# jl6017/AutoURDF

Hardware: AMD Instinct MI355X
Metric: registered frames/sec (N=4096 pts, K=20 clusters) (higher is better)
Workload: dtype f32

## Files before the change

autourdf_amd/csrc/nn_l1.h:

```cpp
#pragma once
#include <type_traits>
#include "creg_dev.h"

namespace creg {

constexpr int NN_TCH = 4096;
constexpr int NN_BLOCK = 512;
typedef float nn_f2 __attribute__((ext_vector_type(2)));

struct NnEpilogueNone {
    __device__ __forceinline__ void finish(int, int, float, float*) const {}
    __device__ __forceinline__ void shift(int) {}
};

template <int QW, typename IdxT, typename Epi>
__device__ __forceinline__ void nn_l1_block(
    const float* A, int na, int sa, const float* B, int nb, int sb,
    float* __restrict__ dA, IdxT* __restrict__ iA, float* __restrict__ dB, IdxT* __restrict__ iB,
    int blocksA, Epi& epi, int bx) {
    extern __shared__ __attribute__((aligned(16))) char smem_raw[];
    float* sX = (float*)smem_raw;
    __shared__ float s_part[NN_BLOCK / 64];
    const int tid = threadIdx.x, lane = tid & 63;
    const int wave = __builtin_amdgcn_readfirstlane(tid >> 6);
// ... 84 lines not shown
        if (dO) { dO[q0 + lane] = mv; iO[q0 + lane] = (IdxT)mi; }
        if constexpr (!std::is_same<Epi, NnEpilogueNone>::value) {
            float tx, ty, tz;
            if (in_lds) { tx = sX[mi]; ty = sX[padded0 + mi]; tz = sX[2 * padded0 + mi]; }
            else { const float* p = T + (size_t)mi * st; tx = p[0]; ty = p[1]; tz = p[2]; }
            epi(dir, q0 + lane, mi, mv, mqx, mqy, mqz, tx, ty, tz, acc);
        }
    }
    if constexpr (!std::is_same<Epi, NnEpilogueNone>::value) {
        acc = wave_sum_fast(acc);
        if (lane == 0) s_part[wave] = acc;
        __syncthreads();
        if (tid == 0) {
            float s = 0.f;
#pragma unroll
            for (int w = 0; w < NN_BLOCK / 64; ++w) s += s_part[w];
            epi.finish(dir, blk, s, nullptr);
        }
    }
}

struct NnBlocks { const float4* ts4; const float* tbox; int nblk; const int* nblk_dev; };

template <int NB, int PPL, typename Epi, bool STOP = false, bool NBDEV = false>
__device__ __forceinline__ void nn_l1_block_pruned(const float* Q, int nq, int sq, NnBlocks tb, int dir, Epi& epi, int blk,
                                                   const int* stop_flag = nullptr, const float* T = nullptr, int st = 0) {
    constexpr int QW = 4;
    int stop = 0;
    if constexpr (STOP) stop = *stop_flag;
    __shared__ float s_partp[NN_BLOCK / 64];
    const int tid = threadIdx.x, lane = tid & 63;
    const int wave = __builtin_amdgcn_readfirstlane(tid >> 6);
    const int q0 = (blk * (NN_BLOCK / 64) + wave) * QW;
    int nblk = tb.nblk;
    if constexpr (NBDEV) nblk = *tb.nblk_dev;
    float lox[NB], loy[NB], loz[NB], hix[NB], hiy[NB], hiz[NB];
#pragma unroll
    for (int g = 0; g < NB; ++g) {
        const float* bx = tb.tbox + (NBDEV ? 64 * g + lane : min(64 * g + lane, nblk - 1));
        constexpr int BP = 64 * NB;
        lox[g] = bx[0]; loy[g] = bx[BP]; loz[g] = bx[2 * BP]; hix[g] = bx[3 * BP]; hiy[g] = bx[4 * BP]; hiz[g] = bx[5 * BP];
    }
    float qx[QW], qy[QW], qz[QW], lb[QW][NB], bd[QW], tx[QW], ty[QW], tz[QW], wb[QW];
    int bi[QW];
    unsigned long long pend[QW][NB];
#pragma unroll
    for (int u = 0; u < QW; ++u) {
        const int qi = min(q0 + u, nq - 1);
        qx[u] = Q[(size_t)qi * sq]; qy[u] = Q[(size_t)qi * sq + 1]; qz[u] = Q[(size_t)qi * sq + 2];
    }
    if constexpr (STOP || NBDEV) {
        stop = __builtin_amdgcn_readfirstlane(stop); nblk = __builtin_amdgcn_readfirstlane(nblk);
#pragma unroll
        for (int u = 0; u < QW; ++u) {
            qx[u] = __int_as_float(__builtin_amdgcn_readfirstlane(__float_as_int(qx[u])));
            qy[u] = __int_as_float(__builtin_amdgcn_readfirstlane(__float_as_int(qy[u])));
            qz[u] = __int_as_float(__builtin_amdgcn_readfirstlane(__float_as_int(qz[u])));
        }
    }
#pragma unroll
    for (int u = 0; u < QW; ++u) {
        float lm = INFINITY;
#pragma unroll
        for (int g = 0; g < NB; ++g) {
            const float ex = fmaxf(fmaxf(lox[g] - qx[u], qx[u] - hix[g]), 0.f);
            const float ey = fmaxf(fmaxf(loy[g] - qy[u], qy[u] - hiy[g]), 0.f);
            const float ez = fmaxf(fmaxf(loz[g] - qz[u], qz[u] - hiz[g]), 0.f);
            const float bound = (ex + ey) + ez;
            lb[u][g] = 64 * g + lane < nblk ? bound : INFINITY;
            lm = __builtin_fminf(lm, lb[u][g]);
        }
        const float m = wave_min_fast(lm);
        bool found = false;
#pragma unroll
        for (int g = 0; g < NB; ++g) {
            const unsigned long long f = __ballot(lb[u][g] == m && 64 * g + lane < nblk);
            pend[u][g] = (!found && f) ? (f & (~f + 1ull)) : 0ull;
            found = found || f != 0ull;
        }
        if (!found) pend[u][0] = 1ull;
        bd[u] = INFINITY; bi[u] = 0x7fffffff; tx[u] = ty[u] = tz[u] = 0.f; wb[u] = INFINITY;
    }
    if (stop) return;
    bool more = true;
    while (more) {
        int b[QW];
        bool act[QW];
#pragma unroll
        for (int u = 0; u < QW; ++u) {
            b[u] = 0; act[u] = false;
#pragma unroll
            for (int g = NB - 1; g >= 0; --g)
                if (pend[u][g]) { b[u] = 64 * g + __builtin_ctzll(pend[u][g]); act[u] = true; }
        }
        float4 v1[QW];
        if constexpr (PPL == 1) {
#pragma unroll
            for (int u = 0; u < QW; ++u) v1[u] = tb.ts4[(size_t)b[u] * 64 + lane];
        }
        more = false;
#pragma unroll
        for (int u = 0; u < QW; ++u) {
            if (act[u]) {
                float4 v[PPL];
                if constexpr (PPL == 1) v[0] = v1[u];
                else {
#pragma unroll
                    for (int k = 0; k < PPL; ++k) v[k] = tb.ts4[((size_t)b[u] * PPL + k) * 64 + lane];
                }
#pragma unroll
                for (int g = 0; g < NB; ++g)
                    if ((b[u] >> 6) == g && lane == (b[u] & 63)) lb[u][g] = INFINITY;
                if constexpr (PPL > 1) {
                    unsigned long long key = ((unsigned long long)__float_as_uint(bd[u]) << 32) | (unsigned)bi[u];
#pragma unroll
                    for (int k = 0; k < PPL; ++k) {
                        const float d = l1_dist(qx[u], qy[u], qz[u], v[k].x, v[k].y, v[k].z);
                        const unsigned long long kk = ((unsigned long long)__float_as_uint(d) << 32) | (unsigned)__float_as_int(v[k].w);
                        key = kk < key ? kk : key;
                    }
                    bd[u] = __uint_as_float((unsigned)(key >> 32)); bi[u] = (int)(unsigned)key;
                } else {
#pragma unroll
                    for (int k = 0; k < PPL; ++k) {
                        const float d = l1_dist(qx[u], qy[u], qz[u], v[k].x, v[k].y, v[k].z);
                        const int oi = __float_as_int(v[k].w);
                        const unsigned long long key = ((unsigned long long)__float_as_uint(bd[u]) << 32) | (unsigned)bi[u];
                        const unsigned long long kk = ((unsigned long long)__float_as_uint(d) << 32) | (unsigned)oi;
                        const bool take = kk < key;
                        bd[u] = take ? d : bd[u]; bi[u] = take ? oi : bi[u];
                        tx[u] = take ? v[k].x : tx[u]; ty[u] = take ? v[k].y : ty[u]; tz[u] = take ? v[k].z : tz[u];
                    }
                }
                wb[u] = wave_min_fast(bd[u]);
#pragma unroll
                for (int g = 0; g < NB; ++g) {
                    pend[u][g] = __ballot(lb[u][g] <= wb[u] && lb[u][g] < INFINITY);
                    more |= pend[u][g] != 0ull;
                }
            }
        }
    }
    float acc = 0.f, mv = 0.f, mqx = 0.f, mqy = 0.f, mqz = 0.f, mtx = 0.f, mty = 0.f, mtz = 0.f;
    int mi = 0;
#pragma unroll
    for (int u = 0; u < QW; ++u) {
        const int i = wave_min_fast(bd[u] == wb[u] ? bi[u] : 0x7fffffff);
        const unsigned long long win = __ballot(bd[u] == wb[u] && bi[u] == i);
        const int src = win ? __builtin_ctzll(win) : 0;
        const float fx = __int_as_float(__builtin_amdgcn_readlane(__float_as_int(tx[u]), src));
        const float fy = __int_as_float(__builtin_amdgcn_readlane(__float_as_int(ty[u]), src));
        const float fz = __int_as_float(__builtin_amdgcn_readlane(__float_as_int(tz[u]), src));
        if (lane == u) { mv = wb[u]; mi = i; mqx = qx[u]; mqy = qy[u]; mqz = qz[u]; mtx = fx; mty = fy; mtz = fz; }
    }
    if constexpr (PPL > 1) {
        if (lane < QW && q0 + lane < nq && mi != 0x7fffffff) { const float* p = T + (size_t)mi * st; mtx = p[0]; mty = p[1]; mtz = p[2]; }
    }
    if (lane < QW && q0 + lane < nq) epi(dir, q0 + lane, mi, mv, mqx, mqy, mqz, mtx, mty, mtz, acc);
    acc = wave_sum_fast(acc);
    if (lane == 0) s_partp[wave] = acc;
    __syncthreads();
    if (tid == 0) {
        float s = 0.f;
#pragma unroll
        for (int w = 0; w < NN_BLOCK / 64; ++w) s += s_partp[w];
        epi.finish(dir, blk, s, nullptr);
    }
}

__device__ __forceinline__ float row_min16(float v) {
    asm("s_nop 4\n\t"
        "v_min_f32_dpp %0, %0, %0 quad_perm:[1,0,3,2] row_mask:0xf bank_mask:0xf\n\ts_nop 1\n\t"
        "v_min_f32_dpp %0, %0, %0 quad_perm:[2,3,0,1] row_mask:0xf bank_mask:0xf\n\ts_nop 1\n\t"
        "v_min_f32_dpp %0, %0, %0 row_half_mirror row_mask:0xf bank_mask:0xf\n\ts_nop 1\n\t"
        "v_min_f32_dpp %0, %0, %0 row_mirror row_mask:0xf bank_mask:0xf\n\ts_nop 1"
        : "+v"(v));
    return v;
}
__device__ __forceinline__ float row_max16(float v) {
    asm("s_nop 4\n\t"
        "v_max_f32_dpp %0, %0, %0 quad_perm:[1,0,3,2] row_mask:0xf bank_mask:0xf\n\ts_nop 1\n\t"
// ... 238 lines not shown
```

autourdf_amd/csrc/train_engine.hip:

```cpp
#include <cfloat>
#include <chrono>
#include <cmath>
#include <cstdlib>
#include <cstring>
#include <type_traits>
#include <vector>
#include "creg_common.h"
#include "nn_l1.h"

#ifndef CREG_L2_IN_BD_DEFAULT
#define CREG_L2_IN_BD_DEFAULT false
#endif

namespace creg {

struct Dims {
    int rot, K, KP, IN, H, HA, HB, H2, OA, OB, NP, NT, epochs;
    float slope;
    int oW1, ob1, oW2, ob2, oW3A, ob3A, oW3B, ob3B, NPAR;
    int nbx, nby;
    int nyb;
    int npb;
    int ppl;
    int nbt, nbp;
    int rows;
};

constexpr int PS_MAXB = 512;

struct Hyper {
    float lr, factor;
    int patience, stop;
};

struct TrainState {
    double lr, sched_best;
    int sched_bad, count, stopped, step;
    float min_loss;
    int epochs_run, best_epoch;
    float step_size, bc2_sqrt;
    float last_loss;
    float next_bc2s;
    double next_bc1;
};

struct Ws {
    float *P, *P1, *AM, *AV;
    float *pose_in, *enc, *x1[2], *h2[2], *head_save, *m2, *gm2;
    float4 *pts4, *y4, *pred4, *ys4, *psl4, *ps4;
    float *ybox, *pbox;
    int* sb;
    int* sgn_x;
    int4* cnt4;
    float *lossp_x, *lossp_y;
    float *g_out, *g_h2;
    TrainState* state;
    double* bc1;
    float* bc2s;
    float *best_m, *best_pred, *loss_hist, *lr_hist, *result;
    int* off;
    Hyper* hyper;
    unsigned long long* ysum;
    int* sync;
};

static_assert(sizeof(Ws) % sizeof(char*) == 0, "Ws must hold pointers only");
__host__ __device__ __forceinline__ Ws ws_shift(Ws W, size_t bytes) {
    char** p = reinterpret_cast<char**>(&W);
#pragma unroll
    for (size_t i = 0; i < sizeof(Ws) / sizeof(char*); ++i) p[i] += bytes;
    return W;
}

constexpr int ROT_Q = 0, ROT_DQ = 1, ROT_6D = 2, ROT_RPY = 3;
constexpr int POSE_IN = 12;
__device__ __forceinline__ float act_f(float v, float slope) { return v > 0.f ? v : v * slope; }
__device__ __forceinline__ float act_grad(float post, float slope) { return post > 0.f ? 1.f : slope; }

__device__ __forceinline__ int seg_of(const int* __restrict__ off, int k, int n) {
    int lo = 0, hi = k;
    while (hi - lo > 1) { const int mid = (lo + hi) >> 1; if (off[mid] <= n) lo = mid; else hi = mid; }
    return lo;
}

constexpr int PREP_MAXB = 64;
struct PrepBatch { const float* m[PREP_MAXB]; const float* y[PREP_MAXB]; const float* pts[PREP_MAXB]; Hyper hy[PREP_MAXB]; };
// ... 39 lines not shown
                nin = 9;
            } else {
                in[0] = tr[0]; in[1] = tr[1]; in[2] = tr[2];
                matrix_to_euler_xyz(R, in + 3);
                nin = 6;
            }
            for (int i = 0; i < POSE_IN; ++i) W.pose_in[POSE_IN * r + i] = in[i];
            float* e = W.enc + (size_t)r * D.IN;
            for (int f = 0; f < 4; ++f) {
                const float mul = (float)(1 << f);
                for (int i = 0; i < nin; ++i) {
                    e[(2 * f) * nin + i] = sinf(mul * in[i]);
                    e[(2 * f + 1) * nin + i] = cosf(mul * in[i]);
                }
            }
        }
        if (threadIdx.x == 0) {
            TrainState s;
            *W.hyper = hy;
            s.lr = (double)hy.lr; s.sched_best = INFINITY; s.sched_bad = 0; s.count = 0; s.stopped = 0;
            s.step = 0; s.min_loss = 1000.f; s.epochs_run = 0; s.best_epoch = -1; s.step_size = 0.f;
            s.bc2_sqrt = 1.f; s.last_loss = NAN;
            s.next_bc1 = 1.0 - 0.9; s.next_bc2s = (float)sqrt(1.0 - 0.999);
            W.state[0] = s; W.state[1] = s;
            for (int i = 0; i < 64; ++i) W.sync[i] = 0;
        }
    }
}

__global__ __launch_bounds__(256) void k_l1(Dims D, Ws W0, int par, size_t bstride) {
    const Ws W = ws_shift(W0, blockIdx.z * bstride);
    const int lane = threadIdx.x & 63;
    const int o = blockIdx.x * 4 + (threadIdx.x >> 6);
    if (o >= D.H) return;
    const float w = lane < D.IN ? W.P[D.oW1 + (size_t)o * D.IN + lane] : 0.f;
    const float w2 = 64 + lane < D.IN ? W.P[D.oW1 + (size_t)o * D.IN + 64 + lane] : 0.f;
    const float b = W.P[D.ob1 + o];
    for (int r = 0; r < D.K; ++r) {
        float t = lane < D.IN ? w * W.enc[(size_t)r * D.IN + lane] : 0.f;
        if (64 + lane < D.IN) t = fmaf(w2, W.enc[(size_t)r * D.IN + 64 + lane], t);
        const float v = wave_sum_fast(t) + b;
        if (lane == 0) (par ? W.x1[1] : W.x1[0])[(size_t)r * D.H + o] = act_f(v, D.slope);
    }
}

typedef float f32x4 __attribute__((ext_vector_type(4)));
constexpr int L2_THREADS = 512;
// ... 89 lines not shown
    else { w = Pc + D.oW3B + (size_t)(o - D.OA) * D.HB; a = h2cur + (size_t)r * D.H2 + D.HA; n = D.HB; }
    float wv[NC], av[NC];
#pragma unroll
    for (int c = 0; c < NC; ++c) { const int i = min(c * 64 + lane, n - 1); wv[c] = w[i]; av[c] = a[i]; }
    const float bias = o < D.OA ? Pc[D.ob3A + o] : Pc[D.ob3B + o - D.OA];
    float wv9[NC], av9[NC], bias9 = 0.f;
    if constexpr (X) {
        const float* w9 = Pc + D.oW3B + (size_t)(8 - D.OA) * D.HB;
        const float* a9 = h2cur + (size_t)r * D.H2 + D.HA;
#pragma unroll
        for (int c = 0; c < NC; ++c) { const int i = min(c * 64 + lane, D.HB - 1); wv9[c] = w9[i]; av9[c] = a9[i]; }
        bias9 = Pc[D.ob3B + 8 - D.OA];
    }
    __builtin_amdgcn_sched_barrier(0);
    const int stopped = W.state[par].stopped;
    float pin[POSE_IN];
#pragma unroll
    for (int i = 0; i < POSE_IN; ++i) pin[i] = W.pose_in[POSE_IN * r + i];
    const int b = W.off[r], e = W.off[r + 1];
    const int BS = 64 * D.ppl;
    const int sb0 = W.sb[r], sb1 = W.sb[r + 1];
    const int s0 = D.npb ? BS * sb0 : 0, s1 = D.npb ? BS * sb1 : 0;
    const float4 p_first = D.npb ? W.psl4[min(s0 + (int)threadIdx.x, BS * D.npb - 1)] : W.pts4[min(b + (int)threadIdx.x, D.NP - 1)];
    {
        float s = 0.f;
#pragma unroll
        for (int c = 0; c < NC; ++c) s = fmaf(c * 64 + lane < n ? wv[c] : 0.f, av[c], s);
        s = wave_sum_fast(s) + bias;
        if (lane == 0 && wave < NO) outs[o] = s;
        if constexpr (X) {
            float s9 = 0.f;
#pragma unroll
            for (int c = 0; c < NC; ++c) s9 = fmaf(c * 64 + lane < D.HB ? wv9[c] : 0.f, av9[c], s9);
            s9 = wave_sum_fast(s9) + bias9;
            if (lane == 0 && wave == 0) outs[8] = s9;
        }
    }
    __syncthreads();
    if (stopped) return;
    if (threadIdx.x == 0) {
        const float* in = pin;
        float R[9], t[3], save[16];
        for (int i = 0; i < 16; ++i) save[i] = 0.f;
        if (D.rot == ROT_6D) {
            for (int i = 0; i < 3; ++i) t[i] = outs[i] + in[i];
            float d6[6];
// ... 21 lines not shown
            for (int i = 0; i < 8; ++i) save[i] = dq[i];
        }
        for (int a = 0; a < 3; ++a) { m2s[4 * a] = R[3 * a]; m2s[4 * a + 1] = R[3 * a + 1]; m2s[4 * a + 2] = R[3 * a + 2]; m2s[4 * a + 3] = t[a]; }
        for (int i = 0; i < 12; ++i) W.m2[16 * r + i] = m2s[i];
        W.m2[16 * r + 12] = 0.f; W.m2[16 * r + 13] = 0.f; W.m2[16 * r + 14] = 0.f; W.m2[16 * r + 15] = 1.f;
        for (int i = 0; i < 16; ++i) W.head_save[16 * r + i] = save[i];
    }
    __syncthreads();
    if (D.npb) {
        __shared__ float wbox[8][6];
        for (int base = s0; base < s1; base += 512) {
            const int sl = base + threadIdx.x;
            const bool in = sl < s1;
            const float4 p = !in ? make_float4(0.f, 0.f, 0.f, __int_as_float(0x7fffffff)) : (base == s0 ? p_first : W.psl4[sl]);
            const int n = __float_as_int(p.w);
            const bool real = n != 0x7fffffff;
            float o[3];
#pragma unroll
            for (int a = 0; a < 3; ++a) o[a] = fmaf(p.z, m2s[4 * a + 2], fmaf(p.y, m2s[4 * a + 1], p.x * m2s[4 * a])) + m2s[4 * a + 3];
            if (real) {
                W.pred4[n] = make_float4(o[0], o[1], o[2], 0.f);
                W.cnt4[n] = make_int4(0, 0, 0, 0);
            }
            if (in) W.ps4[sl] = real ? make_float4(o[0], o[1], o[2], p.w) : make_float4(INFINITY, INFINITY, INFINITY, p.w);
            float bx[6];
#pragma unroll
            for (int a = 0; a < 3; ++a) {
                bx[a] = wave_min_fast(real ? o[a] : INFINITY);
                bx[3 + a] = -wave_min_fast(real ? -o[a] : INFINITY);
            }
            if (D.ppl == 1) {
                if (lane == 0 && in) {
                    float* pb = W.pbox + (sl >> 6);
#pragma unroll
                    for (int a = 0; a < 6; ++a) pb[a * 64 * D.nbp] = bx[a];
                }
            } else {
                if (lane == 0) {
#pragma unroll
                    for (int a = 0; a < 6; ++a) wbox[wave][a] = bx[a];
                }
                __syncthreads();
                if (threadIdx.x < 12) {
                    const int hb = threadIdx.x / 6, a = threadIdx.x % 6;
                    if (base + 256 * hb < s1) {
                        float v = wbox[4 * hb][a];
// ... 215 lines not shown
    const int* stopped;
    __device__ __forceinline__ void shift(int z) {
        const size_t b = (size_t)z * bstride;
        sgn_x = (int*)((char*)sgn_x + b); cnt4 = (int4*)((char*)cnt4 + b);
        lossp_x = (float*)((char*)lossp_x + b); lossp_y = (float*)((char*)lossp_y + b);
        stopped = (const int*)((const char*)stopped + b);
    }
    __device__ __forceinline__ void operator()(int dir, int q, int idx, float d, float qx, float qy, float qz,
                                               float tx, float ty, float tz, float& acc) const {
        if (dir == 0) {
            sgn_x[q] = (qx > tx ? 1 : 0) | (qy > ty ? 2 : 0) | (qz > tz ? 4 : 0);
        } else {
            atomicAdd(&cnt4[idx].x, (qx > tx) ? -1 : 1);
            atomicAdd(&cnt4[idx].y, (qy > ty) ? -1 : 1);
            atomicAdd(&cnt4[idx].z, (qz > tz) ? -1 : 1);
        }
        acc += d;
    }
    __device__ __forceinline__ void finish(int dir, int blk, float s, float*) const { (dir == 0 ? lossp_x : lossp_y)[blk] = s; }
};

template <bool P1, int PPL, int NBT, int NBP>
__global__ __launch_bounds__(NN_BLOCK) void k_nn_plan(const float* A, int na, const float* B, int nb, int blocksA,
                                                      int blocksB, EngineEpi epi, NnBlocks yb, NnBlocks pb, size_t zstride) {
    asm volatile("" :: "s"(A), "s"(na), "s"(B), "s"(nb), "s"(blocksA), "s"(blocksB), "s"(epi.sgn_x), "s"(epi.cnt4), "s"(epi.lossp_x), "s"(epi.lossp_y),
                 "s"(epi.bstride), "s"(epi.stopped), "s"(yb.ts4), "s"(yb.tbox), "s"(yb.nblk), "s"(pb.ts4), "s"(pb.tbox), "s"(pb.nblk_dev), "s"(zstride));
    const int nz = gridDim.x / (blocksA + blocksB);
    int i = blockIdx.x, z, bx;
    if (i < blocksB * nz) { z = i / blocksB; bx = blocksA + (i - z * blocksB); }
    else { i -= blocksB * nz; z = i / blocksA; bx = i - z * blocksA; }
    const size_t zb = z * zstride;
    A = (const float*)((const char*)A + zb);
    B = (const float*)((const char*)B + zb);
    yb.ts4 = (const float4*)((const char*)yb.ts4 + zb);
    yb.tbox = (const float*)((const char*)yb.tbox + zb);
    epi.shift(z);
    if (bx < blocksA) nn_l1_block_pruned<NBT, PPL, EngineEpi, true, false>(A, na, 4, yb, 0, epi, bx, epi.stopped, B, 4);
    else if constexpr (P1) {
        pb.ts4 = (const float4*)((const char*)pb.ts4 + zb);
        pb.tbox = (const float*)((const char*)pb.tbox + zb);
        pb.nblk_dev = (const int*)((const char*)pb.nblk_dev + zb);
        nn_l1_block_pruned<NBP, PPL, EngineEpi, true, true>(B, nb, 4, pb, 1, epi, bx - blocksA, epi.stopped, A, 4);
    } else nn_l1_block<4, int, EngineEpi>(A, na, 4, B, nb, 4, nullptr, nullptr, nullptr, nullptr, blocksA, epi, bx);
}

template <int NBT, int NBP>
__global__ __launch_bounds__(NN_ROWS_BLOCK) void k_nn_rows(const float* A, const float* B, int blocksA, int blocksB, EngineEpi epi, NnBlocks yb, NnBlocks pb,
                                                      size_t zstride) {
    asm volatile("" :: "s"(A), "s"(B), "s"(blocksA), "s"(blocksB), "s"(epi.sgn_x), "s"(epi.cnt4), "s"(epi.lossp_x), "s"(epi.lossp_y),
                 "s"(epi.bstride), "s"(epi.stopped), "s"(yb.ts4), "s"(yb.tbox), "s"(yb.nblk), "s"(pb.ts4), "s"(pb.tbox), "s"(pb.nblk_dev), "s"(zstride));
    const int nz = gridDim.x / (blocksA + blocksB);
    int i = blockIdx.x, z, bx;
    if (i < blocksB * nz) { z = i / blocksB; bx = blocksA + (i - z * blocksB); }
    else { i -= blocksB * nz; z = i / blocksA; bx = i - z * blocksA; }
    const size_t zb = z * zstride;
    A = (const float*)((const char*)A + zb);
    B = (const float*)((const char*)B + zb);
    yb.ts4 = (const float4*)((const char*)yb.ts4 + zb);
    yb.tbox = (const float*)((const char*)yb.tbox + zb);
    pb.ts4 = (const float4*)((const char*)pb.ts4 + zb);
    pb.tbox = (const float*)((const char*)pb.tbox + zb);
    pb.nblk_dev = (const int*)((const char*)pb.nblk_dev + zb);
    epi.shift(z);
    if (bx < blocksA) nn_l1_rows<NBT, EngineEpi, false, true>(pb.ts4, 0, pb.nblk_dev, pb.nblk, yb, 0, epi, bx, epi.stopped, B, epi.lossp_x);
    else nn_l1_rows<NBP, EngineEpi, true, false>(yb.ts4, yb.nblk, nullptr, yb.nblk, pb, 1, epi, bx - blocksA, epi.stopped, A, epi.lossp_y);
// ... 19 lines not shown
        if (N.sched_bad > hy.patience) {
            const double nl = fmax(S.lr * (double)hy.factor, 0.0);
            if (S.lr - nl > 1e-8) N.lr = nl;
            N.sched_bad = 0;
        }
    }
    return N;
}

constexpr int GC_QMAX = 3;
__device__ __forceinline__ void gradc_arrive(const Ws& W) {
    asm volatile("s_waitcnt vmcnt(0)" ::: "memory");
    __syncthreads();
    if (threadIdx.x == 0) __hip_atomic_fetch_add(W.sync, 1, __ATOMIC_RELAXED, __HIP_MEMORY_SCOPE_AGENT);
}
template <bool FUSED>
__device__ __forceinline__ void gradc_role(const Dims& D, const Ws& W, int epoch, int nbx, int nby, int k) {
    __shared__ float red[4][14];
    __shared__ float s_loss;
    __shared__ float s_go[16];
    __shared__ __attribute__((aligned(16))) float s_gh[FUSED ? 256 * GC_QMAX : 4];
    const int tid = threadIdx.x, lane = tid & 63, wv = tid >> 6;
    const TrainState S = W.state[epoch & 1];
    const int handoff_err = W.sync[3];
    const int b0 = W.off[k], e0 = W.off[k + 1];
    const Hyper hy = *W.hyper;
    float a = tid < nbx ? W.lossp_x[tid] : 0.f, b = tid < nby ? W.lossp_y[tid] : 0.f;
    const float m2v = W.m2[16 * k + (tid & 15)];
    float sv[16];
#pragma unroll
    for (int i = 0; i < 16; ++i) sv[i] = W.head_save[16 * k + i];
    const float* h2cur = (epoch & 1) ? W.h2[1] : W.h2[0];
    float w3v[GC_QMAX][8], h2v[GC_QMAX];
#pragma unroll
    for (int q = 0; q < GC_QMAX; ++q) {
        const int o = min(q * 256 + tid, D.H2 - 1);
        const bool isA = o < D.HA;
        const float* Pc = (epoch & 1) ? W.P1 : W.P;
        const float* wb = isA ? Pc + D.oW3A + o : Pc + D.oW3B + (o - D.HA);
        const int stride = isA ? D.HA : D.HB, nj = isA ? D.OA : D.OB;
#pragma unroll
        for (int j = 0; j < 8; ++j) w3v[q][j] = wb[(size_t)min(j, nj - 1) * stride];
        h2v[q] = h2cur[(size_t)k * D.H2 + o];
    }
    asm volatile("" :: "v"(a), "v"(b), "v"(m2v), "v"(sv[0]), "v"(sv[1]), "v"(sv[2]), "v"(sv[3]), "v"(sv[4]), "v"(sv[5]), "v"(sv[6]), "v"(sv[7]),
                 "v"(sv[8]), "v"(sv[9]), "v"(sv[10]), "v"(sv[11]), "v"(sv[12]), "v"(sv[13]), "v"(sv[14]), "v"(sv[15]), "v"(b0), "v"(e0), "v"(hy.lr));
// ... 20 lines not shown
    for (int i = tid + 256; i < nby; i += 256) b += W.lossp_y[i];
    a = wave_sum_fast(a); b = wave_sum_fast(b);
    if (lane == 0) { red[wv][0] = a; red[wv][1] = b; }
    __syncthreads();
    if (tid == 0) {
        const float sa = ((red[0][0] + red[1][0]) + red[2][0]) + red[3][0];
        const float sb = ((red[0][1] + red[1][1]) + red[2][1]) + red[3][1];
        s_loss = sa / (float)D.NP + sb / (float)D.NT;
    }
    __syncthreads();
    const float loss = s_loss;
    TrainState N = advance_state(S, loss, hy, S.next_bc1, S.next_bc2s);
    const bool improved = loss < S.min_loss;
    if (improved) {
        for (int n = b0 + tid; n < e0; n += 256) {
            const float4 p = (n == b0 + tid) ? pr_first : W.pred4[n];
            W.best_pred[3 * (size_t)n] = p.x; W.best_pred[3 * (size_t)n + 1] = p.y; W.best_pred[3 * (size_t)n + 2] = p.z;
        }
        if (tid < 16) W.best_m[16 * k + tid] = m2v;
    }
    if (k == 0 && tid == 0) {
        N.next_bc1 = W.bc1[min(N.step + 1, D.epochs)];
        N.next_bc2s = W.bc2s[min(N.step + 1, D.epochs)];
        W.state[(epoch + 1) & 1] = N;
        W.loss_hist[S.epochs_run] = loss;
        W.lr_hist[S.epochs_run] = (float)S.lr;
        W.result[0] = N.min_loss; W.result[1] = (float)N.epochs_run; W.result[2] = (float)N.lr; W.result[3] = (float)N.best_epoch;
        if constexpr (FUSED) st4_wt((float*)W.sync, 32, make_float4(__int_as_float(N.stopped), N.step_size, N.bc2_sqrt, 0.f));
    }
    if (N.stopped) {
        if constexpr (FUSED) gradc_arrive(W);
        return;
    }
    const float gx = 1.0f / (float)D.NP, gy = 1.0f / (float)D.NT;
    float acc[12];
#pragma unroll
    for (int i = 0; i < 12; ++i) acc[i] = 0.f;
    for (int n = b0 + tid; n < e0; n += 256) {
        const bool first = n == b0 + tid;
        const float4 p = first ? p_first : W.pts4[n];
        const int4 c = first ? c_first : W.cnt4[n];
        const int sb = first ? s_first : W.sgn_x[n];
        const float g[3] = {((sb & 1) ? gx : -gx) + gy * (float)c.x, ((sb & 2) ? gx : -gx) + gy * (float)c.y,
                            ((sb & 4) ? gx : -gx) + gy * (float)c.z};
#pragma unroll
        for (int q = 0; q < 3; ++q) {
// ... 562 lines not shown
    }
    i -= nG * nz;
    const bool roleB = i < nB * nz;
    if (!roleB) i -= nB * nz;
    const int n = roleB ? nB : nD, z = i / n, blk = i - z * n;
    const Ws W = ws_shift(W0, (size_t)z * bstride);
    if (roleB) bwd2_role<KW, X, true>(D, W, epoch, blk, (float*)smem, 0ull);
    else dw_role<true>(D, W, epoch, blk, 0ull);
}

__global__ __launch_bounds__(256) void k_params_home(Dims D, Ws W0, size_t bstride, int sidx, int step0) {
    const Ws W = ws_shift(W0, blockIdx.z * bstride);
    if (((W.state[sidx].step - step0) & 1) == 0) return;
    for (int i = blockIdx.x * 256 + threadIdx.x; i < D.NPAR; i += gridDim.x * 256) W.P[i] = W.P1[i];
}

struct ResumeState { double lr, sched_best; int step, epochs_run, sched_bad, count, best_epoch, stopped; float min_loss; };
__global__ void k_set_state(Dims D, Ws W, ResumeState rs) {
    if (threadIdx.x || blockIdx.x) return;
    TrainState s = W.state[0];
    s.lr = rs.lr; s.sched_best = rs.sched_best; s.sched_bad = rs.sched_bad; s.count = rs.count; s.stopped = rs.stopped; s.step = rs.step;
    s.min_loss = rs.min_loss; s.epochs_run = rs.epochs_run; s.best_epoch = rs.best_epoch;
    s.next_bc1 = W.bc1[min(rs.step + 1, D.epochs)]; s.next_bc2s = W.bc2s[min(rs.step + 1, D.epochs)];
    W.state[0] = s; W.state[1] = s;
    W.sync[1] = (D.H / B2_CB) * rs.step;
    W.result[0] = s.min_loss; W.result[1] = (float)s.epochs_run; W.result[2] = (float)s.lr; W.result[3] = (float)s.best_epoch;
}
__global__ void k_get_state(Ws W, int sidx, double* out) {
    if (threadIdx.x || blockIdx.x) return;
    const TrainState s = W.state[sidx];
    out[0] = s.step; out[1] = s.epochs_run; out[2] = s.lr; out[3] = s.sched_best; out[4] = s.sched_bad; out[5] = s.count;
    out[6] = (double)s.min_loss; out[7] = s.best_epoch; out[8] = s.stopped; out[9] = (double)s.last_loss; out[10] = 0.0; out[11] = 0.0;
}

struct Plan {
    creg_train_shape shape;
    Dims D;
    Ws W;
    char* base;
    size_t bytes;
    hipGraphExec_t gexec;
    bool graph_ready;
    int graph_epochs;
    int B;
    int nz;
    size_t bstride;
    int smem_bd;
// ... 24 lines not shown
    D->H2 = D->HA + D->HB;
    if (sizeof(float) * b2_smem_floats(D->K, D->IN, D->H2) > 160 * 1024) return false;
    int o = 0;
    D->oW1 = o; o += D->H * D->IN; D->ob1 = o; o += D->H;
    D->oW2 = o; o += D->H2 * D->H; D->ob2 = o; o += D->H2;
    D->oW3A = o; o += D->OA * D->HA; D->ob3A = o; o += D->OA;
    D->oW3B = o; o += D->OB * D->HB; D->ob3B = o; o += D->OB;
    D->NPAR = o;
    if (D->H2 % 32 || D->H % B2_CB || D->H2 > 256 * GC_QMAX) return false;
    const NnGrid g = nn_grid(D->NP, D->NT, true, true, 4);
    D->nbx = g.blocksA; D->nby = g.blocksB;
    const bool rows_fit = D->NT <= 16384 && D->NP < 65535 && (D->NP + 63) / 64 + D->K <= PS_MAXB && g.qw == 4;
    const char* rows_env = getenv("CREG_NN_ROWS");
    const bool rows_pays = D->NT > 64 * 64;
    D->rows = s->nn_search == 0 && rows_fit && (rows_env ? rows_env[0] == '1' : rows_pays);
    D->ppl = (D->rows || D->NT <= 64 * 64) ? 1 : 4;
    const int BS = 64 * D->ppl;
    D->nyb = (s->nn_search != 1 && D->NT <= 4 * YS_CHUNK && g.qw == 4) ? (D->NT + BS - 1) / BS : 0;
    D->npb = (D->nyb && D->NP < 65535 && (D->NP + BS - 1) / BS + D->K <= PS_MAXB) ? (D->NP + BS - 1) / BS + D->K : 0;
    const int nt = (D->nyb + 63) / 64, np = (D->npb + 63) / 64;
    D->nbt = nt <= 1 ? 1 : (nt <= 2 ? 2 : 4);
    D->nbp = np <= 2 ? 2 : (np <= 3 ? 3 : (np <= 4 ? 4 : (np <= 5 ? 5 : (np <= 6 ? 6 : 8))));
    if (D->rows) { D->nbx = 4 * D->npb; D->nby = 4 * D->nyb; }
    return true;
}

static size_t carve(const Dims& D, char* base, Ws* W) {
    size_t o = 0;
    auto take = [&](size_t bytes) -> char* { char* r = base ? base + o : nullptr; o = align_up(o + bytes, 256); return r; };
    const size_t f = sizeof(float);
    Ws w;
    w.P = (float*)take(f * D.NPAR); w.P1 = (float*)take(f * D.NPAR); w.AM = (float*)take(f * D.NPAR); w.AV = (float*)take(f * D.NPAR);
    w.pose_in = (float*)take(f * POSE_IN * D.K); w.enc = (float*)take(f * D.K * D.IN);
    w.x1[0] = (float*)take(f * D.KP * D.H); w.x1[1] = (float*)take(f * D.KP * D.H);
    w.h2[0] = (float*)take(f * D.KP * D.H2); w.h2[1] = (float*)take(f * D.KP * D.H2); w.head_save = (float*)take(f * 16 * D.K);
    w.m2 = (float*)take(f * 16 * D.K); w.gm2 = (float*)take(f * 16 * D.K);
    w.pts4 = (float4*)take(sizeof(float4) * D.NP); w.y4 = (float4*)take(sizeof(float4) * D.NT);
    w.pred4 = (float4*)take(sizeof(float4) * D.NP);
    const size_t bs = 64 * (size_t)D.ppl;
    w.ys4 = (float4*)take(sizeof(float4) * bs * (D.nyb ? D.nyb : 1)); w.ybox = (float*)take(f * 6 * 64 * D.nbt);
    w.psl4 = (float4*)take(sizeof(float4) * bs * (D.npb ? D.npb : 1)); w.ps4 = (float4*)take(sizeof(float4) * bs * (D.npb ? D.npb : 1));
    w.pbox = (float*)take(f * 6 * 64 * D.nbp); w.sb = (int*)take(sizeof(int) * (D.K + 1));
    w.sgn_x = (int*)take(sizeof(int) * D.NP);
    w.cnt4 = (int4*)take(sizeof(int4) * D.NP);
    w.lossp_x = (float*)take(f * D.nbx); w.lossp_y = (float*)take(f * D.nby);
    w.g_out = (float*)take(f * 16 * D.KP); w.g_h2 = (float*)take(f * D.KP * D.H2);
    w.state = (TrainState*)take(sizeof(TrainState) * 2);
    w.bc1 = (double*)take(sizeof(double) * (D.epochs + 1)); w.bc2s = (float*)take(f * (D.epochs + 1));
    w.best_m = (float*)take(f * 16 * D.K); w.best_pred = (float*)take(f * 3 * D.NP);
    w.loss_hist = (float*)take(f * D.epochs); w.lr_hist = (float*)take(f * D.epochs); w.result = (float*)take(f * 4);
    w.off = (int*)take(sizeof(int) * (D.K + 1)); w.hyper = (Hyper*)take(sizeof(Hyper));
    w.sync = (int*)take(sizeof(int) * 64);
    w.ysum = (unsigned long long*)take(sizeof(unsigned long long) * 4);
    if (W) *W = w;
    return o;
}

template <typename F>
static void by_nc(int H, F f) {
    switch (H / 64) {
        case 1: f(std::integral_constant<int, 1>{}); break;
        case 2: f(std::integral_constant<int, 2>{}); break;
        case 4: f(std::integral_constant<int, 4>{}); break;
        default: f(std::integral_constant<int, 8>{}); break;
    }
}
static void launch_l2(Plan* P, int par, hipStream_t s) {
    const Dims& D = P->D; const Ws& W = P->W;
    by_nc(D.H, [&](auto nc) {
        hipLaunchKernelGGL((k_l2<decltype(nc)::value>), dim3(D.H2 / 16, 1, P->nz), dim3(L2_THREADS), 0, s, D, W, par, P->bstride); });
}
static void launch_head(Plan* P, int par, hipStream_t s) {
    const Dims& D = P->D; const Ws& W = P->W;
    by_nc(D.H, [&](auto nc) {
        if (D.OA + D.OB > 8) hipLaunchKernelGGL((k_head<decltype(nc)::value, true>), dim3(D.K, 1, P->nz), dim3(512), 0, s, D, W, par, P->bstride);
        else hipLaunchKernelGGL((k_head<decltype(nc)::value>), dim3(D.K, 1, P->nz), dim3(512), 0, s, D, W, par, P->bstride);
// ... 41 lines not shown
        auto go = [&](auto kern) {
            hipLaunchKernelGGL(kern, grid, dim3(NN_ROWS_BLOCK), 0, s, (const float*)W.pred4, (const float*)W.y4, blocksA, blocksB, epi, yb, pb, bstride);
        };
        auto pick_p = [&](auto nbt) {
            constexpr int NBT = decltype(nbt)::value;
            switch (D.nbp) {
                case 2: go(k_nn_rows<NBT, 2>); break;
                case 3: go(k_nn_rows<NBT, 3>); break;
                case 4: go(k_nn_rows<NBT, 4>); break;
                case 5: go(k_nn_rows<NBT, 5>); break;
                case 6: go(k_nn_rows<NBT, 6>); break;
                default: go(k_nn_rows<NBT, 8>); break;
            }
        };
        switch (D.nbt) {
            case 1: pick_p(std::integral_constant<int, 1>{}); break;
            case 2: pick_p(std::integral_constant<int, 2>{}); break;
            default: pick_p(std::integral_constant<int, 4>{}); break;
        }
    } else if (D.nyb) {
        const NnGrid g = nn_grid(D.NP, D.NT, true, true, 4);
        const NnBlocks yb{W.ys4, W.ybox, D.nyb, nullptr}, pb{W.ps4, W.pbox, 0, W.sb + D.K};
        const dim3 grid((g.blocksA + g.blocksB) * nz);
        auto go = [&](auto kern, int smem) {
            hipLaunchKernelGGL(kern, grid, dim3(NN_BLOCK), smem, s, (const float*)W.pred4, D.NP, (const float*)W.y4, D.NT,
                               g.blocksA, g.blocksB, epi, yb, pb, bstride);
        };
        auto pick_p = [&](auto ppl, auto nbt) {
            constexpr int PPL = decltype(ppl)::value, NBT = decltype(nbt)::value;
            if (!D.npb) { go(k_nn_plan<false, PPL, NBT, 2>, g.smem); return; }
            switch (D.nbp) {
                case 2: go(k_nn_plan<true, PPL, NBT, 2>, 0); break;
                case 3: go(k_nn_plan<true, PPL, NBT, 3>, 0); break;
                case 4: go(k_nn_plan<true, PPL, NBT, 4>, 0); break;
                case 5: go(k_nn_plan<true, PPL, NBT, 5>, 0); break;
                case 6: go(k_nn_plan<true, PPL, NBT, 6>, 0); break;
                default: go(k_nn_plan<true, PPL, NBT, 8>, 0); break;
            }
        };
        auto pick_t = [&](auto ppl) {
            switch (D.nbt) {
                case 1: pick_p(ppl, std::integral_constant<int, 1>{}); break;
                case 2: pick_p(ppl, std::integral_constant<int, 2>{}); break;
                default: pick_p(ppl, std::integral_constant<int, 4>{}); break;
            }
        };
        if (D.ppl == 1) pick_t(std::integral_constant<int, 1>{}); else pick_t(std::integral_constant<int, 4>{});
    } else {
        launch_nn_l1<int>((const float*)W.pred4, D.NP, 4, (const float*)W.y4, D.NT, 4, nullptr, nullptr, nullptr, nullptr,
// ... 550 lines not shown
    for (auto& e : ev) (void)hipEventDestroy(e);
    return CREG_OK;
}

#ifdef CREG_BD_STAMPS
extern "C" int creg_debug_bd_stamps(double* out) {
    BdStamps* z = new BdStamps;
    if (hipMemcpyFromSymbol(z, HIP_SYMBOL(g_bd_st), sizeof(*z)) != hipSuccess) { delete z; return CREG_EHIP; }
    for (int i = 0; i < 24; ++i) out[i] = 0.0;
    int n = 0;
    for (int sl = 0; sl < 256; ++sl) {
        if (z->first[sl] == ~0ull || !z->endB[sl] || !z->endD[sl]) continue;
        ++n;
        const double f = (double)z->first[sl];
        out[0] += ((double)(z->endB[sl] > z->endD[sl] ? z->endB[sl] : z->endD[sl]) - f) / 100.0;
        out[1] += ((double)z->startB[sl] - f) / 100.0; out[2] += ((double)z->endB[sl] - f) / 100.0;
        out[3] += ((double)z->startD[sl] - f) / 100.0; out[4] += ((double)z->endD[sl] - f) / 100.0;
    }
    for (int i = 0; i < 5; ++i) out[i] /= n ? n : 1;
    out[5] = n ? (double)z->blocks[0] / n : 0; out[6] = n ? (double)z->blocks[1] / n : 0; out[7] = n;
    for (int r = 0; r < 2; ++r)
        for (int k = 0; k < 8; ++k) out[8 + 8 * r + k] = z->blocks[r] ? (double)z->phase[r][k] / (double)z->blocks[r] / 100.0 : 0.0;
    delete z;
    return CREG_OK;
}
#endif

#ifdef CREG_NN_STATS
extern "C" int creg_debug_nn_stats(unsigned long long* out8, int reset) {
    CREG_HIP(hipMemcpyFromSymbol(out8, HIP_SYMBOL(creg::g_nn_stats), sizeof(unsigned long long) * 8));
    if (reset) { unsigned long long z[8] = {0}; CREG_HIP(hipMemcpyToSymbol(HIP_SYMBOL(creg::g_nn_stats), z, sizeof(z))); }
    return CREG_OK;
}
#endif

#ifdef CREG_NN_WAVE_STAMPS
extern "C" long long creg_debug_nn_waves(unsigned long long* out, long long cap, int reset) {
    static unsigned n[creg::NN_WAVE_SHARDS * 32];
    if (hipMemcpyFromSymbol(n, HIP_SYMBOL(creg::g_nn_wave_n), sizeof(n)) != hipSuccess) return -1;
    long long total = 0;
    if (out && cap > 0) {
        std::vector<creg::NnWaveRec> h((size_t)creg::NN_WAVE_CAP);
        if (hipMemcpyFromSymbol(h.data(), HIP_SYMBOL(creg::g_nn_wave), sizeof(creg::NnWaveRec) * (size_t)creg::NN_WAVE_CAP) != hipSuccess) return -1;
        for (unsigned sh = 0; sh < creg::NN_WAVE_SHARDS; ++sh) {
            const unsigned m = n[32 * sh] < creg::NN_WAVE_PER ? n[32 * sh] : creg::NN_WAVE_PER;
            for (unsigned i = 0; i < m && total < cap; ++i, ++total) {
// ... 287 lines not shown
```

Baseline: 165.5.

## Certify nearest-neighbor matches across epochs to skip pruned search

```diff
diff --git a/autourdf_amd/csrc/nn_l1.h b/autourdf_amd/csrc/nn_l1.h
--- a/autourdf_amd/csrc/nn_l1.h
+++ b/autourdf_amd/csrc/nn_l1.h
@@ -130,12 +130,32 @@
 
 struct NnBlocks { const float4* ts4; const float* tbox; int nblk; const int* nblk_dev; };
 
-template <int NB, int PPL, typename Epi, bool STOP = false, bool NBDEV = false>
+struct NnCert {
+    float4* ref;
+    int* j;
+    const int* ok;
+    const double* s;
+    const unsigned* delta;
+    int nt;
+};
+__device__ __forceinline__ double nn_cert_s(int ok, double s_prev, unsigned delta_bits) {
+    return ok ? (s_prev + (double)__uint_as_float(delta_bits)) * (1.0 + 0x1p-50) : 0.0;
+}
+#ifdef CREG_NN_CERT_STATS
+__device__ unsigned long long g_nn_cert_stats[8];
+#endif
+
+template <int NB, int PPL, typename Epi, bool STOP = false, bool NBDEV = false, bool CERT = false>
 __device__ __forceinline__ void nn_l1_block_pruned(const float* Q, int nq, int sq, NnBlocks tb, int dir, Epi& epi, int blk,
-                                                   const int* stop_flag = nullptr, const float* T = nullptr, int st = 0) {
+                                                   const int* stop_flag = nullptr, const float* T = nullptr, int st = 0, NnCert cert = {}) {
     constexpr int QW = 4;
+    static_assert(!CERT || PPL == 1, "certified matches: one point per lane");
     int stop = 0;
     if constexpr (STOP) stop = *stop_flag;
+    int cok = 0;
+    double cs_prev = 0.0;
+    unsigned cdelta = 0u;
+    if constexpr (CERT) { cok = *cert.ok; cs_prev = *cert.s; cdelta = *cert.delta; }
     __shared__ float s_partp[NN_BLOCK / 64];
     const int tid = threadIdx.x, lane = tid & 63;
     const int wave = __builtin_amdgcn_readfirstlane(tid >> 6);
@@ -166,8 +186,43 @@
             qz[u] = __int_as_float(__builtin_amdgcn_readfirstlane(__float_as_int(qz[u])));
         }
     }
+    unsigned long long cmask = 0ull;
+    const double cS = CERT ? nn_cert_s(cok, cs_prev, cdelta) : 0.0;
+    float b2[QW];
+    float cd = 0.f, ctx = 0.f, cty = 0.f, ctz = 0.f;
+    int cj = 0;
+    if constexpr (CERT) {
+        if (cok) {
+            const int cq = min(q0 + min(lane, QW - 1), nq - 1);
+            const float4 r = cert.ref[cq];
+            const int j0 = cert.j[cq];
+            const float4 qv = ((const float4*)Q)[cq];
+            const bool jin = j0 >= 0 && j0 < cert.nt;
+            const float4 tv = ((const float4*)T)[jin ? j0 : 0];
+            const float d = l1_dist(qv.x, qv.y, qv.z, tv.x, tv.y, tv.z);
+            const double A = dir == 0 ? (fabs((double)qv.x - (double)r.x) + fabs((double)qv.y - (double)r.y)) + fabs((double)qv.z - (double)r.z)
+                                      : cS - __hiloint2double(__float_as_int(r.y), __float_as_int(r.x));
+            const double R = (double)r.w * (1.0 - 0x1p-20) - A * (1.0 + 0x1p-40);
+            cmask = __ballot(lane < QW && q0 + lane < nq && jin && r.w <= 0x1p126f && (double)d < R);
+            cd = d; cj = j0; ctx = tv.x; cty = tv.y; ctz = tv.z;
+        }
+#ifdef CREG_NN_CERT_STATS
+        if (lane == 0 && !stop) {
+            const int nv = min(QW, nq - q0), nc = __builtin_popcountll(cmask);
+            atomicAdd(&g_nn_cert_stats[4 * dir], 1ull); atomicAdd(&g_nn_cert_stats[4 * dir + 1], (unsigned long long)nv);
+            atomicAdd(&g_nn_cert_stats[4 * dir + 2], (unsigned long long)nc);
+            if (nc == nv) atomicAdd(&g_nn_cert_stats[4 * dir + 3], 1ull);
+        }
+#endif
+    }
 #pragma unroll
     for (int u = 0; u < QW; ++u) {
+        b2[u] = INFINITY;
+        if (CERT && ((cmask >> u) & 1ull)) {
+#pragma unroll
+            for (int g = 0; g < NB; ++g) { lb[u][g] = INFINITY; pend[u][g] = 0ull; }
+            continue;
+        }
         float lm = INFINITY;
 #pragma unroll
         for (int g = 0; g < NB; ++g) {
@@ -190,7 +245,7 @@
         bd[u] = INFINITY; bi[u] = 0x7fffffff; tx[u] = ty[u] = tz[u] = 0.f; wb[u] = INFINITY;
     }
     if (stop) return;
-    bool more = true;
+    bool more = !CERT || cmask != (1ull << QW) - 1;
     while (more) {
         int b[QW];
         bool act[QW];
@@ -236,6 +291,7 @@
                         const unsigned long long key = ((unsigned long long)__float_as_uint(bd[u]) << 32) | (unsigned)bi[u];
                         const unsigned long long kk = ((unsigned long long)__float_as_uint(d) << 32) | (unsigned)oi;
                         const bool take = kk < key;
+                        if constexpr (CERT) b2[u] = take ? bd[u] : __builtin_fminf(b2[u], d);
                         bd[u] = take ? d : bd[u]; bi[u] = take ? oi : bi[u];
                         tx[u] = take ? v[k].x : tx[u]; ty[u] = take ? v[k].y : ty[u]; tz[u] = take ? v[k].z : tz[u];
                     }
@@ -249,10 +305,14 @@
             }
         }
     }
-    float acc = 0.f, mv = 0.f, mqx = 0.f, mqy = 0.f, mqz = 0.f, mtx = 0.f, mty = 0.f, mtz = 0.f;
+    float acc = 0.f, mv = 0.f, mqx = 0.f, mqy = 0.f, mqz = 0.f, mtx = 0.f, mty = 0.f, mtz = 0.f, cL = 0.f;
     int mi = 0;
 #pragma unroll
     for (int u = 0; u < QW; ++u) {
+        if (CERT && ((cmask >> u) & 1ull)) {
+            if (lane == u) { mv = cd; mi = cj; mqx = qx[u]; mqy = qy[u]; mqz = qz[u]; mtx = ctx; mty = cty; mtz = ctz; }
+            continue;
+        }
         const int i = wave_min_fast(bd[u] == wb[u] ? bi[u] : 0x7fffffff);
         const unsigned long long win = __ballot(bd[u] == wb[u] && bi[u] == i);
         const int src = win ? __builtin_ctzll(win) : 0;
@@ -260,11 +320,25 @@
         const float fy = __int_as_float(__builtin_amdgcn_readlane(__float_as_int(ty[u]), src));
         const float fz = __int_as_float(__builtin_amdgcn_readlane(__float_as_int(tz[u]), src));
         if (lane == u) { mv = wb[u]; mi = i; mqx = qx[u]; mqy = qy[u]; mqz = qz[u]; mtx = fx; mty = fy; mtz = fz; }
+        if constexpr (CERT) {
+            float lm = lane == src ? b2[u] : bd[u];
+#pragma unroll
+            for (int g = 0; g < NB; ++g) lm = __builtin_fminf(lm, lb[u][g]);
+            lm = wave_min_fast(lm);
+            if (lane == u) cL = lm;
+        }
     }
     if constexpr (PPL > 1) {
         if (lane < QW && q0 + lane < nq && mi != 0x7fffffff) { const float* p = T + (size_t)mi * st; mtx = p[0]; mty = p[1]; mtz = p[2]; }
     }
     if (lane < QW && q0 + lane < nq) epi(dir, q0 + lane, mi, mv, mqx, mqy, mqz, mtx, mty, mtz, acc);
+    if constexpr (CERT) {
+        if (lane < QW && q0 + lane < nq && !((cmask >> lane) & 1ull)) {
+            cert.j[q0 + lane] = mi;
+            cert.ref[q0 + lane] = dir == 0 ? make_float4(mqx, mqy, mqz, cL)
+                                           : make_float4(__int_as_float(__double2loint(cS)), __int_as_float(__double2hiint(cS)), 0.f, cL);
+        }
+    }
     acc = wave_sum_fast(acc);
     if (lane == 0) s_partp[wave] = acc;
     __syncthreads();
diff --git a/autourdf_amd/csrc/train_engine.hip b/autourdf_amd/csrc/train_engine.hip
--- a/autourdf_amd/csrc/train_engine.hip
+++ b/autourdf_amd/csrc/train_engine.hip
@@ -10,6 +10,9 @@
 
 #ifndef CREG_L2_IN_BD_DEFAULT
 #define CREG_L2_IN_BD_DEFAULT false
+#endif
+#ifndef CREG_NN_CERT
+#define CREG_NN_CERT 1
 #endif
 
 namespace creg {
@@ -24,6 +27,7 @@
     int ppl;
     int nbt, nbp;
     int rows;
+    int cert;
 };
 
 constexpr int PS_MAXB = 512;
@@ -42,6 +46,8 @@
     float last_loss;
     float next_bc2s;
     double next_bc1;
+    double cert_s;
+    int cert_ok;
 };
 
 struct Ws {
@@ -62,6 +68,9 @@
     Hyper* hyper;
     unsigned long long* ysum;
     int* sync;
+    float4 *cref0, *cref1;
+    int *cj0, *cj1;
+    unsigned* cdel;
 };
 
 static_assert(sizeof(Ws) % sizeof(char*) == 0, "Ws must hold pointers only");
@@ -147,7 +156,9 @@
             s.step = 0; s.min_loss = 1000.f; s.epochs_run = 0; s.best_epoch = -1; s.step_size = 0.f;
             s.bc2_sqrt = 1.f; s.last_loss = NAN;
             s.next_bc1 = 1.0 - 0.9; s.next_bc2s = (float)sqrt(1.0 - 0.999);
+            s.cert_s = 0.0; s.cert_ok = 0;
             W.state[0] = s; W.state[1] = s;
+            W.cdel[0] = 0u; W.cdel[1] = 0u;
             for (int i = 0; i < 64; ++i) W.sync[i] = 0;
         }
     }
@@ -283,6 +294,8 @@
     const int sb0 = W.sb[r], sb1 = W.sb[r + 1];
     const int s0 = D.npb ? BS * sb0 : 0, s1 = D.npb ? BS * sb1 : 0;
     const float4 p_first = D.npb ? W.psl4[min(s0 + (int)threadIdx.x, BS * D.npb - 1)] : W.pts4[min(b + (int)threadIdx.x, D.NP - 1)];
+    float4 po_first = make_float4(0.f, 0.f, 0.f, 0.f);
+    if (CREG_NN_CERT && D.cert) po_first = W.ps4[min(s0 + (int)threadIdx.x, BS * D.npb - 1)];
     {
         float s = 0.f;
 #pragma unroll
@@ -350,6 +363,12 @@
                 W.pred4[n] = make_float4(o[0], o[1], o[2], 0.f);
                 W.cnt4[n] = make_int4(0, 0, 0, 0);
             }
+            if (CREG_NN_CERT && D.cert) {
+                const float4 po = base == s0 ? po_first : (in ? W.ps4[sl] : make_float4(0.f, 0.f, 0.f, 0.f));
+                const float dd = real ? ((fabsf(o[0] - po.x) + fabsf(o[1] - po.y)) + fabsf(o[2] - po.z)) * (1.f + 0x1p-20f) : 0.f;
+                const int mx = -wave_min_fast(-(int)__float_as_uint(dd));
+                if (lane == 0 && mx) atomicMax(W.cdel + par, (unsigned)mx);
+            }
             if (in) W.ps4[sl] = real ? make_float4(o[0], o[1], o[2], p.w) : make_float4(INFINITY, INFINITY, INFINITY, p.w);
             float bx[6];
 #pragma unroll
@@ -611,9 +630,13 @@
 
 template <bool P1, int PPL, int NBT, int NBP>
 __global__ __launch_bounds__(NN_BLOCK) void k_nn_plan(const float* A, int na, const float* B, int nb, int blocksA,
-                                                      int blocksB, EngineEpi epi, NnBlocks yb, NnBlocks pb, size_t zstride) {
+                                                      int blocksB, EngineEpi epi, NnBlocks yb, NnBlocks pb, size_t zstride, NnCert c0, NnCert c1) {
+    constexpr bool CERT = CREG_NN_CERT && P1 && PPL == 1;
     asm volatile("" :: "s"(A), "s"(na), "s"(B), "s"(nb), "s"(blocksA), "s"(blocksB), "s"(epi.sgn_x), "s"(epi.cnt4), "s"(epi.lossp_x), "s"(epi.lossp_y),
                  "s"(epi.bstride), "s"(epi.stopped), "s"(yb.ts4), "s"(yb.tbox), "s"(yb.nblk), "s"(pb.ts4), "s"(pb.tbox), "s"(pb.nblk_dev), "s"(zstride));
+    if constexpr (CERT)
+        asm volatile("" :: "s"(c0.ref), "s"(c0.j), "s"(c0.ok), "s"(c0.s), "s"(c0.delta), "s"(c0.nt), "s"(c1.ref), "s"(c1.j), "s"(c1.ok), "s"(c1.s), "s"(c1.delta),
+                     "s"(c1.nt));
     const int nz = gridDim.x / (blocksA + blocksB);
     int i = blockIdx.x, z, bx;
     if (i < blocksB * nz) { z = i / blocksB; bx = blocksA + (i - z * blocksB); }
@@ -624,12 +647,19 @@
     yb.ts4 = (const float4*)((const char*)yb.ts4 + zb);
     yb.tbox = (const float*)((const char*)yb.tbox + zb);
     epi.shift(z);
-    if (bx < blocksA) nn_l1_block_pruned<NBT, PPL, EngineEpi, true, false>(A, na, 4, yb, 0, epi, bx, epi.stopped, B, 4);
-    else if constexpr (P1) {
+    auto cshift = [&](NnCert& c) {
+        c.ref = (float4*)((char*)c.ref + zb); c.j = (int*)((char*)c.j + zb); c.ok = (const int*)((const char*)c.ok + zb);
+        c.s = (const double*)((const char*)c.s + zb); c.delta = (const unsigned*)((const char*)c.delta + zb);
+    };
+    if (bx < blocksA) {
+        if constexpr (CERT) cshift(c0);
+        nn_l1_block_pruned<NBT, PPL, EngineEpi, true, false, CERT>(A, na, 4, yb, 0, epi, bx, epi.stopped, B, 4, c0);
+    } else if constexpr (P1) {
         pb.ts4 = (const float4*)((const char*)pb.ts4 + zb);
         pb.tbox = (const float*)((const char*)pb.tbox + zb);
         pb.nblk_dev = (const int*)((const char*)pb.nblk_dev + zb);
-        nn_l1_block_pruned<NBP, PPL, EngineEpi, true, true>(B, nb, 4, pb, 1, epi, bx - blocksA, epi.stopped, A, 4);
+        if constexpr (CERT) cshift(c1);
+        nn_l1_block_pruned<NBP, PPL, EngineEpi, true, true, CERT>(B, nb, 4, pb, 1, epi, bx - blocksA, epi.stopped, A, 4, c1);
     } else nn_l1_block<4, int, EngineEpi>(A, na, 4, B, nb, 4, nullptr, nullptr, nullptr, nullptr, blocksA, epi, bx);
 }
 
@@ -695,6 +725,7 @@
     __shared__ __attribute__((aligned(16))) float s_gh[FUSED ? 256 * GC_QMAX : 4];
     const int tid = threadIdx.x, lane = tid & 63, wv = tid >> 6;
     const TrainState S = W.state[epoch & 1];
+    const unsigned cdelta = (CREG_NN_CERT && D.cert) ? W.cdel[epoch & 1] : 0u;
     const int handoff_err = W.sync[3];
     const int b0 = W.off[k], e0 = W.off[k + 1];
     const Hyper hy = *W.hyper;
@@ -761,6 +792,11 @@
     if (k == 0 && tid == 0) {
         N.next_bc1 = W.bc1[min(N.step + 1, D.epochs)];
         N.next_bc2s = W.bc2s[min(N.step + 1, D.epochs)];
+        if (CREG_NN_CERT && D.cert) {
+            N.cert_s = nn_cert_s(S.cert_ok, S.cert_s, cdelta);
+            N.cert_ok = 1;
+            W.cdel[(epoch + 1) & 1] = 0u;
+        }
         W.state[(epoch + 1) & 1] = N;
         W.loss_hist[S.epochs_run] = loss;
         W.lr_hist[S.epochs_run] = (float)S.lr;
@@ -1369,7 +1405,9 @@
     s.lr = rs.lr; s.sched_best = rs.sched_best; s.sched_bad = rs.sched_bad; s.count = rs.count; s.stopped = rs.stopped; s.step = rs.step;
     s.min_loss = rs.min_loss; s.epochs_run = rs.epochs_run; s.best_epoch = rs.best_epoch;
     s.next_bc1 = W.bc1[min(rs.step + 1, D.epochs)]; s.next_bc2s = W.bc2s[min(rs.step + 1, D.epochs)];
+    s.cert_s = 0.0; s.cert_ok = 0;
     W.state[0] = s; W.state[1] = s;
+    W.cdel[0] = 0u; W.cdel[1] = 0u;
     W.sync[1] = (D.H / B2_CB) * rs.step;
     W.result[0] = s.min_loss; W.result[1] = (float)s.epochs_run; W.result[2] = (float)s.lr; W.result[3] = (float)s.best_epoch;
 }
@@ -1440,6 +1478,7 @@
     D->nbt = nt <= 1 ? 1 : (nt <= 2 ? 2 : 4);
     D->nbp = np <= 2 ? 2 : (np <= 3 ? 3 : (np <= 4 ? 4 : (np <= 5 ? 5 : (np <= 6 ? 6 : 8))));
     if (D->rows) { D->nbx = 4 * D->npb; D->nby = 4 * D->nyb; }
+    D->cert = CREG_NN_CERT && D->nyb && D->npb && !D->rows && D->ppl == 1;
     return true;
 }
 
@@ -1470,6 +1509,9 @@
     w.off = (int*)take(sizeof(int) * (D.K + 1)); w.hyper = (Hyper*)take(sizeof(Hyper));
     w.sync = (int*)take(sizeof(int) * 64);
     w.ysum = (unsigned long long*)take(sizeof(unsigned long long) * 4);
+    w.cref0 = (float4*)take(sizeof(float4) * (D.cert ? D.NP : 1)); w.cj0 = (int*)take(sizeof(int) * (D.cert ? D.NP : 1));
+    w.cref1 = (float4*)take(sizeof(float4) * (D.cert ? D.NT : 1)); w.cj1 = (int*)take(sizeof(int) * (D.cert ? D.NT : 1));
+    w.cdel = (unsigned*)take(sizeof(unsigned) * 2);
     if (W) *W = w;
     return o;
 }
@@ -1557,9 +1599,11 @@
         const NnGrid g = nn_grid(D.NP, D.NT, true, true, 4);
         const NnBlocks yb{W.ys4, W.ybox, D.nyb, nullptr}, pb{W.ps4, W.pbox, 0, W.sb + D.K};
         const dim3 grid((g.blocksA + g.blocksB) * nz);
+        const NnCert c0{W.cref0, W.cj0, &W.state[par].cert_ok, &W.state[par].cert_s, W.cdel + par, D.NT};
+        const NnCert c1{W.cref1, W.cj1, &W.state[par].cert_ok, &W.state[par].cert_s, W.cdel + par, D.NP};
         auto go = [&](auto kern, int smem) {
             hipLaunchKernelGGL(kern, grid, dim3(NN_BLOCK), smem, s, (const float*)W.pred4, D.NP, (const float*)W.y4, D.NT,
-                               g.blocksA, g.blocksB, epi, yb, pb, bstride);
+                               g.blocksA, g.blocksB, epi, yb, pb, bstride, c0, c1);
         };
         auto pick_p = [&](auto ppl, auto nbt) {
             constexpr int PPL = decltype(ppl)::value, NBT = decltype(nbt)::value;
@@ -2156,6 +2200,14 @@
     for (int r = 0; r < 2; ++r)
         for (int k = 0; k < 8; ++k) out[8 + 8 * r + k] = z->blocks[r] ? (double)z->phase[r][k] / (double)z->blocks[r] / 100.0 : 0.0;
     delete z;
+    return CREG_OK;
+}
+#endif
+
+#ifdef CREG_NN_CERT_STATS
+extern "C" int creg_debug_nn_cert_stats(unsigned long long* out8, int reset) {
+    CREG_HIP(hipMemcpyFromSymbol(out8, HIP_SYMBOL(creg::g_nn_cert_stats), sizeof(unsigned long long) * 8));
+    if (reset) { unsigned long long z[8] = {0}; CREG_HIP(hipMemcpyToSymbol(HIP_SYMBOL(creg::g_nn_cert_stats), z, sizeof(z))); }
     return CREG_OK;
 }
 #endif
```

After: 154.9, median of 2. 6.4% lower.
